# isarandi/metrabs

Measured on NVIDIA H100. Metric: crops/sec, higher is better.
Workload: dtype bf16

## Files before the change

### metrabs_b200/csrc/engine.cu

```cuda
#include "../../include/metrabs_b200.h"

#include <dlfcn.h>

#include <algorithm>
#include <cmath>
#include <cstdarg>
#include <cstdio>
#include <cstdlib>
#include <cstring>
#include <iterator>
#include <map>
#include <string>
#include <vector>

#include "common.cuh"
#include "conv_simt.cuh"
#include "decode.cuh"
#include "tc_gemm.cuh"
#include "tc_fmb.cuh"
#include "tc_tf32.cuh"
#include "dw_tma.cuh"
#include "multiperson.cuh"

using namespace mtb;
// ... 759 lines not shown
    if (pl.ok && pl.n_rb <= kPoolSlices) {
      op.dw_kernel = DW_TMA_DIL;
      op.dw_plan = pl;
      op.pool_slices = pl.n_rb;
    }
    return;
  }
  if (dw5x5_eligible(op)) {
    if (!is_tc16(h)) return;
    if (op.act != ACT_SILU) {
      op.dw_kernel = DW_5X5_16B;
      return;
    }
    op.dw_kernel = DW_5X5_POOL_16B;
    const int strips = op.Hout * ((op.Wout + kDw5OW - 1) / kDw5OW);
    const int groups = dw5_pool_shape(op.Cout).groups;
    op.pool_slices = std::min((strips + groups - 1) / groups, kPoolSlices);
    return;
  }
  if (!dw_strip_eligible(op)) return;
  if (is_tc16(h)) {
    if (op.stride == 1 && op.Hin == op.Hout && op.Win == op.Wout) {
      const DwTmaPlan pl = dw_tma_plan(op.Hout, op.Wout);
      if (pl.ok && pl.n_rb <= kPoolSlices) {
        op.dw_kernel = DW_TMA;
        op.dw_plan = pl;
        op.pool_slices = pl.n_rb;
        return;
      }
    }
    op.dw_kernel = DW_STRIP_16B;
  } else if (h->cfg.precision == MTB_PRECISION_TF32X3) {
    op.dw_kernel = DW_STRIP_F32;
  } else {
    return;
  }
  const int strips = op.Hout * ((op.Wout + kDwOW - 1) / kDwOW);
  op.pool_slices = std::min((strips + 7) / 8, kPoolSlices);
}

int op_class(const Op& op) {
  switch (op.type) {
    case OP_STEM: return KC_STEM;
    case OP_DW: return KC_DWCONV;
    case OP_POOL: return KC_POOL;
    case OP_MAXPOOL: return KC_OTHER;
    default: break;
  }
  if (op.small_io) return KC_SE_FC;
  if (op.fmb.ready) return KC_FMB;
  if (op.tc.ready) return KC_TC_GEMM;
  if (op.tc32.ready) return KC_TC32;
  return KC_IGEMM_SIMT;
}

double op_weight_bytes(const Op& op) {
  if (op.type == OP_POOL || op.type == OP_MAXPOOL) return 0.0;
  return (double)op.R * op.S * (op.depthwise ? 1 : op.Cin) * op.Cout * (op.tc.ready ? 2.0 : 4.0);
}

double op_bytes(const mtb_handle* h, const Op& op, int B) {
  const double es = op.small_io ? 4.0 : (double)elem_size(h);
  double in = (double)B * op.Hin * op.Win * op.Cin * (op.type == OP_STEM ? 4.0 : es);
  double out = (double)B * op.Hout * op.Wout * op.Cout * es;
  if (op.type == OP_POOL) out = (double)B * op.Cout * 4.0;
  double res = op.res_buf != BUF_NONE ? out : 0.0;
  return in + out + res + op_weight_bytes(op);
}

bool stem_fast_enabled() {
  static int v = -1;
  if (v < 0) {
    const char* e = getenv("MTB_STEM_FAST");
    v = (e && e[0] == '0') ? 0 : 1;
  }
  return v == 1;
}

template <typename T>
int run_op_t(mtb_handle* h, const Op& op, const float* crops, int B, const Workspace& ws, void* features,
             cudaStream_t st) {
  constexpr bool k16 = sizeof(T) == 2;
  if constexpr (k16) {
    if (op.type == OP_CONV && op.tc.ready && op.scale_buf != BUF_NONE) {
      void* x = buf_ptr(ws, op.in_buf, features);
      const double bytes = 2.0 * B * op.Hin * op.Win * op.Cin * elem_size(h);
      ProfScope ps(h, KC_SE_SCALE, 0.0, bytes, st, false);
      const char* e = tc_se_scale_launch<T>(x, (const float*)buf_ptr(ws, op.scale_buf, features), B, op.Hin * op.Win, op.Cin, st);
      if (e) return fail(h, MTB_ERR_CUDA, "se scale %s: %s", op.name.c_str(), e);
      h->launches++;
    }
  }
  ProfScope prof(h, op_class(op), op.flops * B, op_bytes(h, op, B), st);
  switch (op.type) {
    case OP_STEM: {
      StemParams p;
      p.in = crops;
      p.out = buf_ptr(ws, op.out_buf, features); p.w = op.d_w; p.bias = op.d_bias;
      for (int i = 0; i < 3; ++i) { p.pre_scale[i] = op.pre_scale[i]; p.pre_shift[i] = op.pre_shift[i]; }
      p.pre_scale[3] = 1.f; p.pre_shift[3] = 0.f;
      p.B = B; p.Hin = op.Hin; p.Win = op.Win; p.Cin = op.Cin; p.Hout = op.Hout; p.Wout = op.Wout; p.Cout = op.Cout;
      p.R = op.R; p.S = op.S; p.stride = op.stride; p.pad_t = op.pad_t; p.pad_l = op.pad_l; p.act = op.act;
      size_t smem = ((size_t)op.R * op.S * op.Cin + 1) * op.Cout * 4;
      const size_t pixels = (size_t)B * op.Hout * op.Wout;
      const bool effnet_stem = op.R == 3 && op.S == 3 && op.Cin == 3 && op.stride == 2 && stem_fast_enabled();
      if (effnet_stem && op.Cout == 32) launch_k(stem3x3s2_kernel<T, 32>, dim3(grid_for(pixels, 128)), dim3(128), (size_t)28 * 32 * 4, st, p);
      else if (effnet_stem && op.Cout == 24) launch_k(stem3x3s2_kernel<T, 24>, dim3(grid_for(pixels, 128)), dim3(128), (size_t)28 * 24 * 4, st, p);
      else if (op.Cout % 32 == 0) launch_k(stem_conv_wide_kernel<T, 32>, dim3(grid_for(pixels * (op.Cout / 32), 128)), dim3(128), smem, st, p);
      else if (op.Cout % 24 == 0) launch_k(stem_conv_wide_kernel<T, 24>, dim3(grid_for(pixels * (op.Cout / 24), 128)), dim3(128), smem, st, p);
      else if (op.Cout % 16 == 0) launch_k(stem_conv_wide_kernel<T, 16>, dim3(grid_for(pixels * (op.Cout / 16), 128)), dim3(128), smem, st, p);
      else launch_k(stem_conv_kernel<T>, dim3(grid_for(pixels * (op.Cout / 4), 256)), dim3(256), smem, st, p);
      h->launches++;
      break;
    }
    case OP_CONV:
    case OP_DW:
    case OP_MAXPOOL: {
      ConvParams p;
      p.in = buf_ptr(ws, op.in_buf, features);
      p.out = buf_ptr(ws, op.out_buf, features);
      p.res = buf_ptr(ws, op.res_buf, features);
      p.a_scale = (const float*)buf_ptr(ws, op.scale_buf, features);
      p.w = op.d_w; p.bias = op.d_bias;
      p.B = B; p.Hin = op.Hin; p.Win = op.Win; p.Cin = op.Cin; p.Hout = op.Hout; p.Wout = op.Wout; p.Cout = op.Cout;
      p.R = op.R; p.S = op.S; p.stride = op.stride; p.dil = op.dil; p.pad_t = op.pad_t; p.pad_l = op.pad_l; p.act = op.act;
      p.res_first = op.res_first ? 1 : 0;
      if (op.type == OP_DW) {
        float* pooled = op.fused_pool ? (float*)buf_ptr(ws, BUF_SMALL0, features) : nullptr;
        if (op.dw_kernel == DW_TMA || op.dw_kernel == DW_TMA_DIL || op.dw_kernel == DW_STRIP_16B) {
          if constexpr (!k16) {
            return fail(h, MTB_ERR_CUDA, "depthwise %s: 16-bit kernel chosen for fp32 storage", op.name.c_str());
          } else if (op.dw_kernel == DW_TMA || op.dw_kernel == DW_TMA_DIL) {
            const char* e = dw_tma_launch<T>(op.dw_maps, op.dw_plan, p.in, p.out, op.d_w, op.d_bias, pooled, B, op.Hout, op.Wout,
                                             op.Cout, op.pad_t, op.pad_l, op.act, op.dw_kernel == DW_TMA ? 1 : op.dil, st);
            if (e) return fail(h, MTB_ERR_CUDA, "depthwise (TMA) launch %s: %s", op.name.c_str(), e);
          } else {
            const dim3 grid((op.Cout / 8 + 31) / 32, op.pool_slices, B), block(32, 8);
            const cudaError_t e = dw_dispatch<ACT_SILU, ACT_RELU, ACT_HSWISH>(op, [&](auto s, auto a) {
              return launch_k(dwconv3x3_pool_16b_kernel<T, s, a, kDwOW>, grid, block, 0, st, p, pooled);
            });
            if (e != cudaSuccess) return fail(h, MTB_ERR_CUDA, "depthwise launch %s: %s", op.name.c_str(), cudaGetErrorString(e));
          }
        } else if (op.dw_kernel == DW_STRIP_F32) {
          const dim3 grid((op.Cout / 4 + 31) / 32, op.pool_slices, B), block(32, 8);
          const cudaError_t e = dw_dispatch<ACT_SILU, ACT_RELU, ACT_HSWISH>(op, [&](auto s, auto a) {
            return launch_k(dwconv3x3_pool_f32_kernel<s, a, kDwOW>, grid, block, 0, st, p, pooled);
          });
          if (e != cudaSuccess) return fail(h, MTB_ERR_CUDA, "depthwise launch %s: %s", op.name.c_str(), cudaGetErrorString(e));
        } else if (op.dw_kernel == DW_5X5_16B || op.dw_kernel == DW_5X5_POOL_16B) {
          if constexpr (!k16) {
            return fail(h, MTB_ERR_CUDA, "depthwise %s: 16-bit kernel chosen for fp32 storage", op.name.c_str());
          } else {
            cudaError_t e;
            if (op.dw_kernel == DW_5X5_16B) {
              const size_t items = (size_t)B * op.Hout * ((op.Wout + kDw5OW - 1) / kDw5OW) * (op.Cout / 8);
              const dim3 grid(grid_for(items, 256));
              e = dw_dispatch<ACT_RELU, ACT_HSWISH>(op, [&](auto s, auto a) {
                return launch_k(dwconv5x5_16b_kernel<T, s, a, kDw5OW>, grid, dim3(256), 0, st, p, nullptr);
              });
            } else {
              const Dw5PoolShape sh = dw5_pool_shape(op.Cout);
              const dim3 grid(sh.chunks, op.pool_slices, B), block(sh.cb * sh.groups);
              e = dw_dispatch<ACT_SILU>(op, [&](auto s, auto a) {
                return launch_k(dwconv5x5_16b_kernel<T, s, a, kDw5OW, true>, grid, block, 0, st, p, pooled);
              });
            }
            if (e != cudaSuccess) return fail(h, MTB_ERR_CUDA, "depthwise launch %s: %s", op.name.c_str(), cudaGetErrorString(e));
          }
        } else {
          size_t total = (size_t)B * op.Hout * op.Wout * (op.Cout / 4);
          launch_k(dwconv_kernel<T>, dim3(grid_for(total, 256)), dim3(256), 0, st, p);
        }
      } else if (op.type == OP_MAXPOOL) {
        size_t total = (size_t)B * op.Hout * op.Wout * (op.Cout / 4);
        launch_k(maxpool_kernel<T>, dim3(grid_for(total, 256)), dim3(256), 0, st, p);
      } else if (op.small_io) {
        if (op.pool_src > 0 && h->ops[op.pool_src].fused_pool) {
          p.a_splits = h->ops[op.pool_src - 1].pool_slices;
          p.a_split_stride = (size_t)B * op.Cin;
        }
        float* final_out = (float*)p.out;
        if (op.ksplit > 1) {
          p.ksplit = op.ksplit;
          p.out = buf_ptr(ws, BUF_SMALL0 + 2, features);
        }
        cudaError_t e = launch_conv_igemm<float, float>(p, st);
        if (e == cudaSuccess && op.ksplit > 1) {
          const int n = B * op.Cout;
          launch_k(se_reduce_kernel, dim3((n + 255) / 256), dim3(256), 0, st, (const float*)p.out, (const float*)op.d_bias, final_out, n,
                   op.Cout, op.ksplit, op.act);
          h->launches++;
          e = cudaGetLastError();
        }
        if (e != cudaSuccess) return fail(h, MTB_ERR_CUDA, "launch %s: %s", op.name.c_str(), cudaGetErrorString(e));
      } else if (op.tc.ready) {
        if constexpr (!k16) return fail(h, MTB_ERR_CUDA, "%s: tensor-core weights in an fp32 mode", op.name.c_str());
        else {
          const char* e = tc_conv_launch<T>(op.tc, p, op.res_first, st);
          if (e) return fail(h, MTB_ERR_CUDA, "tensor-core launch %s: %s", op.name.c_str(), e);
        }
      } else if (op.tc32.ready) {
        const char* e = tc32_conv_launch(op.tc32, p, op.res_first, st);
        if (e) return fail(h, MTB_ERR_CUDA, "3xTF32 launch %s: %s", op.name.c_str(), e);
      } else {
        cudaError_t e = launch_conv_igemm<T, T>(p, st);
        if (e != cudaSuccess) return fail(h, MTB_ERR_CUDA, "launch %s: %s", op.name.c_str(), cudaGetErrorString(e));
      }
      h->launches++;
      break;
    }
    case OP_POOL: {
      dim3 grid((op.Cin + 127) / 128, B), block(32, 8);
      launch_k(pool_mean_kernel<T>, dim3(grid), dim3(block), 0, st, (const T*)buf_ptr(ws, op.in_buf, features),
                                                   (float*)buf_ptr(ws, op.out_buf, features), op.Hin * op.Win, op.Cin);
      h->launches++;
      break;
    }
  }
  cudaError_t e = cudaGetLastError();
  if (e != cudaSuccess) return fail(h, MTB_ERR_CUDA, "launch %s: %s", op.name.c_str(), cudaGetErrorString(e));
  return MTB_OK;
}

int run_op(mtb_handle* h, const Op& op, const float* crops, int B, const Workspace& ws, void* features, cudaStream_t st) {
  if (op.type == OP_POOL && op.fused_pool) return MTB_OK;
  return with_storage(h, [&](auto* tag) { return run_op_t<std::remove_pointer_t<decltype(tag)>>(h, op, crops, B, ws, features, st); });
}

int run_fused_block(mtb_handle* h, const Op& a, const Op& b, int B, const Workspace& ws, void* features, cudaStream_t st) {
  const void* in = buf_ptr(ws, a.in_buf, features);
  void* out = buf_ptr(ws, b.out_buf, features);
  const double bytes = 2.0 * B * a.Hin * a.Win * (a.Cin + b.Cout) + 2.0 * (9.0 * a.Cin * a.Cout + (double)b.Cin * b.Cout);
  ProfScope prof(h, KC_FMB, (a.flops + b.flops) * B, bytes, st);
  const char* e = with_storage16(h, [&](auto* tag) {
    return fmb_launch<std::remove_pointer_t<decltype(tag)>>(a.fmb, in, out, B, a.Hin, a.Win, a.pad_t, a.pad_l, b.res_buf != BUF_NONE, st);
  });
  if (e) return fail(h, MTB_ERR_CUDA, "fused FusedMBConv launch %s: %s", a.name.c_str(), e);
  h->launches++;
  return MTB_OK;
}

int run_ops_range(mtb_handle* h, size_t first, size_t last, const float* crops, int B, const Workspace& ws, void* features,
                  cudaStream_t st) {
  for (size_t k = first; k < last; ++k) {
    h->prof_cur_op = (int)k;
    int rc;
    if (h->ops[k].fmb.ready && k + 1 < last) {
      rc = run_fused_block(h, h->ops[k], h->ops[k + 1], B, ws, features, st);
      ++k;
    } else {
      rc = run_op(h, h->ops[k], crops, B, ws, features, st);
    }
    if (rc) return rc;
  }
  h->prof_cur_op = -1;
  return MTB_OK;
}

int run_backbone(mtb_handle* h, const float* crops, int B, Workspace& ws, void* features, cudaStream_t st) {
  return run_ops_range(h, 0, h->ops.size(), crops, B, ws, features, st);
}

int check_common(mtb_handle* h, int B, size_t ws_bytes, const void* workspace) {
  if (!h) return fail(nullptr, MTB_ERR_INVALID_ARG, "null handle");
  if (!h->finalized) return fail(h, MTB_ERR_NOT_FINALIZED, "mtb_finalize_weights has not been called");
  if (B <= 0) return fail(h, MTB_ERR_INVALID_ARG, "batch must be positive (got %d)", B);
  if (!workspace || ws_bytes < layout(h, B, nullptr).total)
    return fail(h, MTB_ERR_WORKSPACE, "workspace too small: need %zu bytes for batch %d, got %zu",
                layout(h, B, nullptr).total, B, ws_bytes);
  return MTB_OK;
}

DecodeScale make_scale(const mtb_config& c) {
  DecodeScale s;
  int last = c.proc_side - 1;
  int last_rc = last - (last % c.stride_test);
  float add = 0.f;
  if (c.centered_stride) add += (float)(c.stride_test / 2);
  if (c.legacy_centered_stride_bug) add += (float)(c.stride_test / 2);
  s.img_mul = (float)last_rc;
// ... 1108 lines not shown
```

### metrabs_b200/csrc/tc_gemm.cuh

```cuda
#pragma once
#include <cuda.h>

#include <algorithm>
#include <cstdio>
#include <cstdlib>
#include <cstring>
#include <string>
#include <vector>

#include "common.cuh"
#include "conv_simt.cuh"
#include "decode.cuh"
#include "wgmma.cuh"

namespace mtb {

__device__ __forceinline__ uint32_t smem_u32(const void* p) { return (uint32_t)__cvta_generic_to_shared(p); }

__device__ __forceinline__ void mbar_init(uint64_t* bar, uint32_t count) {
  asm volatile("mbarrier.init.shared::cta.b64 [%0], %1;" ::"r"(smem_u32(bar)), "r"(count));
}
__device__ __forceinline__ void mbar_expect_tx(uint64_t* bar, uint32_t bytes) {
  asm volatile("mbarrier.arrive.expect_tx.shared::cta.b64 _, [%0], %1;" ::"r"(smem_u32(bar)), "r"(bytes) : "memory");
}
__device__ __forceinline__ void mbar_arrive(uint64_t* bar) {
  asm volatile("mbarrier.arrive.shared::cta.b64 _, [%0];" ::"r"(smem_u32(bar)) : "memory");
}
__device__ __forceinline__ bool mbar_try_wait(uint64_t* bar, uint32_t parity) {
  uint32_t ok;
  asm volatile(
      "{\n"
      ".reg .pred P1;\n"
      "mbarrier.try_wait.parity.shared::cta.b64 P1, [%1], %2;\n"
      "selp.u32 %0, 1, 0, P1;\n"
      "}\n"
      : "=r"(ok)
      : "r"(smem_u32(bar)), "r"(parity)
      : "memory");
  return ok != 0;
}
__device__ __forceinline__ void mbar_wait(uint64_t* bar, uint32_t parity) {
  if (mbar_try_wait(bar, parity)) return;
  const long long t0 = clock64();
  while (!mbar_try_wait(bar, parity))
    if (clock64() - t0 > 8000000000LL) __trap();
}
__device__ __forceinline__ void fence_barrier_init() { asm volatile("fence.mbarrier_init.release.cluster;" ::: "memory"); }
__device__ __forceinline__ void fence_proxy_async() { asm volatile("fence.proxy.async.shared::cta;" ::: "memory"); }
__device__ __forceinline__ void wg_sync(int wg) { asm volatile("bar.sync %0, 128;" ::"r"(1 + wg) : "memory"); }

__device__ __forceinline__ void tma_load_2d(void* dst, const CUtensorMap* map, uint64_t* bar, int c0, int c1) {
  asm volatile(
      "cp.async.bulk.tensor.2d.shared::cluster.global.tile.mbarrier::complete_tx::bytes [%0], [%1, {%3, %4}], [%2];" ::"r"(
          smem_u32(dst)),
      "l"(map), "r"(smem_u32(bar)), "r"(c0), "r"(c1)
      : "memory");
}
__device__ __forceinline__ void tma_load_4d(void* dst, const CUtensorMap* map, uint64_t* bar, int c0, int c1, int c2, int c3) {
  asm volatile(
      "cp.async.bulk.tensor.4d.shared::cluster.global.tile.mbarrier::complete_tx::bytes [%0], [%1, {%3, %4, %5, %6}], [%2];" ::"r"(
          smem_u32(dst)),
      "l"(map), "r"(smem_u32(bar)), "r"(c0), "r"(c1), "r"(c2), "r"(c3)
      : "memory");
}
__device__ __forceinline__ void tma_store_2d(const CUtensorMap* map, const void* src, int c0, int c1) {
  asm volatile("cp.async.bulk.tensor.2d.global.shared::cta.bulk_group [%0, {%2, %3}], [%1];" ::"l"(map), "r"(smem_u32(src)), "r"(c0),
               "r"(c1)
               : "memory");
}
__device__ __forceinline__ void tma_store_4d(const CUtensorMap* map, const void* src, int c0, int c1, int c2, int c3) {
  asm volatile("cp.async.bulk.tensor.4d.global.shared::cta.bulk_group [%0, {%2, %3, %4, %5}], [%1];" ::"l"(map), "r"(smem_u32(src)),
               "r"(c0), "r"(c1), "r"(c2), "r"(c3)
               : "memory");
}
__device__ __forceinline__ void bulk_commit() { asm volatile("cp.async.bulk.commit_group;" ::: "memory"); }
__device__ __forceinline__ void bulk_wait_read() { asm volatile("cp.async.bulk.wait_group.read 0;" ::: "memory"); }
__device__ __forceinline__ void bulk_wait() { asm volatile("cp.async.bulk.wait_group 0;" ::: "memory"); }
__device__ __forceinline__ void tma_prefetch_desc(const CUtensorMap* map) {
  asm volatile("prefetch.tensormap [%0];" ::"l"(map) : "memory");
}

template <int RB>
__device__ __forceinline__ uint64_t gmma_desc(uint32_t smem_addr) {
  uint64_t d = 0;
  d |= (uint64_t)((smem_addr & 0x3FFFF) >> 4);
  d |= (uint64_t)1 << 16;
  d |= (uint64_t)((8 * RB) >> 4) << 32;
  d |= (uint64_t)(RB == 128 ? 1 : 2) << 62;
  return d;
}

constexpr int TC_BM = 128, TC_BK = 64;
constexpr int TC_A_BYTES = TC_BM * TC_BK * 2;
constexpr int TC_THREADS = 288;
constexpr int TC_CONSUMER_WARPS = 8;
constexpr int TC_TILE_W = 16, TC_TILE_H = 8;
constexpr int TCP_THREADS = 384;

template <int BN>
struct TcRing {
  static constexpr int stages = BN >= 128 ? 5 : 8;
  static constexpr int stage_bytes = TC_A_BYTES + BN * TC_BK * 2;
  static constexpr int slab_cols = BN < 64 ? BN : 64;
  static constexpr int out_bytes = TC_BM * BN * 2;
  static constexpr int out_off = stages * stage_bytes;
  static constexpr int bar_off = out_off + 2 * out_bytes;
  static constexpr int smem_bytes = bar_off + 256  + 1024 ;
};

struct TcConvParams {
  const void* res;
  const float* bias;
  void* out;
  int mode;
  int Hin, Win;
  int M;
  int Cout, Cin;
  int kchunks, taps;
  int Hout, Wout, tiles_w, tiles_h, pad_t, pad_l, S, stride, dil;
  int m_tiles, n_tiles;
};

template <int R>
__device__ __forceinline__ void setmaxnreg_dec() { asm volatile("setmaxnreg.dec.sync.aligned.u32 %0;" ::"n"(R)); }
template <int R>
__device__ __forceinline__ void setmaxnreg_inc() { asm volatile("setmaxnreg.inc.sync.aligned.u32 %0;" ::"n"(R)); }
__device__ __forceinline__ void named_bar_sync(int id) { asm volatile("bar.sync %0, 256;" ::"r"(id) : "memory"); }
__device__ __forceinline__ void named_bar_arrive(int id) { asm volatile("bar.arrive %0, 256;" ::"r"(id) : "memory"); }

__device__ __forceinline__ float tanh_approx(float x) {
  float y;
  asm("tanh.approx.f32 %0, %1;" : "=f"(y) : "f"(x));
  return y;
}
template <int ACT, typename T = __nv_bfloat16>
__device__ __forceinline__ float tc_act(float x) {
  if constexpr (ACT == ACT_SILU && is_f16<T>) {
    return silu_f16out(x);
  } else if constexpr (ACT == ACT_SILU) {
    float h = 0.5f * x;
    return fmaf(h, tanh_approx(h), h);
  } else if constexpr (ACT == ACT_RELU) {
    return fmaxf(x, 0.0f);
  } else if constexpr (ACT == ACT_HSWISH) {
    return x * __saturatef(fmaf(x, 1.0f / 6.0f, 0.5f));
  } else {
    return x;
  }
}
__device__ __forceinline__ bool tile_row_offset(int mode, int m_blk, int r, int M, int Cout, int tiles_w, int tiles_h, int Hout, int Wout,
                                                size_t& off) {
  if (mode == 0) {
    const int m = m_blk * TC_BM + r;
    off = (size_t)m * Cout;
    return m < M;
  }
  const int tw = m_blk % tiles_w, th = (m_blk / tiles_w) % tiles_h, b = m_blk / (tiles_w * tiles_h);
  const int oh = th * TC_TILE_H + (r >> 4), ow = tw * TC_TILE_W + (r & 15);
  off = ((size_t)(b * Hout + oh) * Wout + ow) * Cout;
  return oh < Hout && ow < Wout;
// ... 14 lines not shown
template <typename P>
__device__ __forceinline__ void tma_load_tap_boxes(uint8_t* dst, int box_bytes, const CUtensorMap* map, uint64_t* bar, const P& p, int m_blk,
                                                   int kc) {
  const int tw = m_blk % p.tiles_w, th = (m_blk / p.tiles_w) % p.tiles_h, b = m_blk / (p.tiles_w * p.tiles_h);
  for (int s = 0; s < p.S; ++s)
    tma_load_4d(dst + s * box_bytes, map, bar, kc * TC_BK, tw * TC_TILE_W - p.pad_l + s, th * TC_TILE_H - p.pad_t, b);
}

template <typename T, int ACT, int RES, int BN>
__device__ __forceinline__ void tc_tile_epilogue(const float* acc, uint8_t* stg, const CUtensorMap* tmO, const TcConvParams& p, int m_blk,
                                                 int n_blk, int c) {
  constexpr int SW = BN < 64 ? BN : 64, RB = SW * 2;
  typedef typename Pair16<T>::type T2;
  const T* __restrict__ res = (const T*)p.res;
  const int warp = (threadIdx.x >> 5) & 3, lane = threadIdx.x & 31;
  const bool leader = (threadIdx.x & 127) == 0;
  if (leader) bulk_wait_read();
  wg_sync(2 + c);
  const int c0 = n_blk * BN + 2 * (lane & 3);
#pragma unroll
  for (int mh = 0; mh < 2; ++mh) {
    const float* accm = acc + mh * (BN / 2);
#pragma unroll
    for (int h = 0; h < 2; ++h) {
      const int r = mh * 64 + warp * 16 + (lane >> 2) + 8 * h;
      size_t off = 0;
      if constexpr (RES != 0) {
        if (!tile_row_offset(p.mode, m_blk, r, p.M, p.Cout, p.tiles_w, p.tiles_h, p.Hout, p.Wout, off)) continue;
      }
      const uint32_t swz = RB == 128 ? (uint32_t)(r & 7) : (uint32_t)((r >> 1) & 3);
      constexpr int JB = BN / 8 < 8 ? BN / 8 : 8;
#pragma unroll
      for (int j0 = 0; j0 < BN / 8; j0 += JB) {
        T2 rv2[RES != 0 ? JB : 1];
        if constexpr (RES != 0) {
#pragma unroll
          for (int jj = 0; jj < JB; ++jj)
            if (c0 + 8 * (j0 + jj) < p.Cout) rv2[jj] = *reinterpret_cast<const T2*>(res + off + c0 + 8 * (j0 + jj));
        }
#pragma unroll
        for (int j = j0; j < j0 + JB; ++j) {
          const int cc = c0 + 8 * j;
          if (cc >= p.Cout) break;
          const float2 bv = __ldg(reinterpret_cast<const float2*>(p.bias + cc));
          float o0 = accm[4 * j + 2 * h] + bv.x, o1 = accm[4 * j + 2 * h + 1] + bv.y;
          if constexpr (RES != 0) {
            const float2 rv = Pair16<T>::unpack(rv2[j - j0]);
            if constexpr (RES == 2) {
              o0 = tc_act<ACT, T>(o0 + rv.x);
              o1 = tc_act<ACT, T>(o1 + rv.y);
            } else {
              o0 = tc_act<ACT, T>(o0) + rv.x;
              o1 = tc_act<ACT, T>(o1) + rv.y;
            }
          } else {
            o0 = tc_act<ACT, T>(o0);
            o1 = tc_act<ACT, T>(o1);
          }
          const int col = 8 * j + 2 * (lane & 3), cs = col % SW;
          const uint32_t o = (uint32_t)(col / SW) * (TC_BM * RB) + (uint32_t)r * RB + ((((uint32_t)cs >> 3) ^ swz) << 4) + (cs & 7) * 2;
          *reinterpret_cast<T2*>(stg + o) = Pair16<T>::pack(o0, o1);
        }
      }
    }
  }
  fence_proxy_async();
  wg_sync(2 + c);
  if (leader) {
#pragma unroll
    for (int sl = 0; sl < BN / SW; ++sl) {
      const int col0 = n_blk * BN + sl * SW;
      if (col0 >= p.Cout) break;
      if (p.mode == 0) {
        tma_store_2d(tmO, stg + sl * TC_BM * RB, col0, m_blk * TC_BM);
      } else {
        const int tw = m_blk % p.tiles_w, th = (m_blk / p.tiles_w) % p.tiles_h, b = m_blk / (p.tiles_w * p.tiles_h);
        tma_store_4d(tmO, stg + sl * TC_BM * RB, col0, tw * TC_TILE_W, th * TC_TILE_H, b);
      }
    }
    bulk_commit();
  }
}

template <typename T, int ACT, int RES, int BN>
__global__ void __launch_bounds__(TCP_THREADS, 1)
tc_conv_kernel(const __grid_constant__ CUtensorMap tmA, const __grid_constant__ CUtensorMap tmB, const __grid_constant__ CUtensorMap tmO,
               const TcConvParams p) {
  using Ring = TcRing<BN>;
  constexpr int STAGES = Ring::stages;
  extern __shared__ uint8_t tc_smem_raw[];
  uint8_t* smem = (uint8_t*)(((uintptr_t)tc_smem_raw + 1023) & ~(uintptr_t)1023);
  uint64_t* full = (uint64_t*)(smem + Ring::bar_off);
  uint64_t* empty = full + STAGES;

  const int wg = threadIdx.x >> 7, lane = threadIdx.x & 31;
  if (threadIdx.x == 0) {
    tma_prefetch_desc(&tmA);
    tma_prefetch_desc(&tmB);
    tma_prefetch_desc(&tmO);
    for (int i = 0; i < STAGES; ++i) {
      mbar_init(&full[i], 1);
      mbar_init(&empty[i], 4);
    }
    fence_barrier_init();
  }
  __syncthreads();

  const int tiles = p.m_tiles * p.n_tiles;
  const int num_kb = p.taps * p.kchunks;
  if (wg == 0) {
    setmaxnreg_dec<40>();
    if (threadIdx.x == 0) {
      int it = 0;
      for (int t = blockIdx.x; t < tiles; t += gridDim.x) {
        const int m_blk = t / p.n_tiles, n_blk = t - m_blk * p.n_tiles;
        for (int kb = 0; kb < num_kb; ++kb, ++it) {
          const int s = it % STAGES;
          mbar_wait(&empty[s], ((it / STAGES) & 1) ^ 1);
          uint8_t* sa = smem + s * Ring::stage_bytes;
          const int tap = kb / p.kchunks, kc = kb - tap * p.kchunks;
          mbar_expect_tx(&full[s], Ring::stage_bytes);
          tma_load_a_tile<TC_BK>(sa, &tmA, &full[s], p, m_blk, kb);
          tma_load_2d(sa + TC_A_BYTES, &tmB, &full[s], tap * p.Cin + kc * TC_BK, n_blk * BN);
        }
      }
    }
    return;
  }
  setmaxnreg_inc<232>();
  const int c = wg - 1;
  for (int i = c, t = blockIdx.x + c * gridDim.x; t < tiles; i += 2, t += 2 * gridDim.x) {
    const int m_blk = t / p.n_tiles, n_blk = t - m_blk * p.n_tiles;
    float acc[BN];
#pragma unroll
    for (int q = 0; q < BN; ++q) acc[q] = 0.f;
    if (t != (int)blockIdx.x) named_bar_sync(1 + c);
    int it = i * num_kb, prev = -1;
    for (int kb = 0; kb < num_kb; ++kb, ++it) {
      const int s = it % STAGES;
      mbar_wait(&full[s], (it / STAGES) & 1);
      const uint32_t a = smem_u32(smem + s * Ring::stage_bytes);
      const uint32_t b = smem_u32(smem + s * Ring::stage_bytes + TC_A_BYTES);
      wgmma_fence();
#pragma unroll
      for (int k = 0; k < TC_BK / 16; ++k) {
        const uint64_t db = gmma_desc<128>(b + 32 * k);
        wgmma_16b<T, BN>(acc, gmma_desc<128>(a + 32 * k), db, (uint32_t)(kb | k));
        wgmma_16b<T, BN>(acc + BN / 2, gmma_desc<128>(a + 64 * 128 + 32 * k), db, (uint32_t)(kb | k));
      }
      wgmma_commit();
      wgmma_wait<1>();
      if (prev >= 0) {
        __syncwarp();
        if (lane == 0) mbar_arrive(&empty[prev]);
      }
      prev = s;
    }
    wgmma_wait<0>();
    wgmma_fence_regs<BN>(acc);
    __syncwarp();
    if (lane == 0) mbar_arrive(&empty[prev]);
    if (t + (int)gridDim.x < tiles) named_bar_arrive(2 - c);
    tc_tile_epilogue<T, ACT, RES, BN>(acc, smem + Ring::out_off + c * Ring::out_bytes, &tmO, p, m_blk, n_blk, c);
  }
  if ((threadIdx.x & 127) == 0) bulk_wait();
}

template <int CK>
struct Tc3x3Smem {
  static constexpr int RB = CK * 2;
  static constexpr int w_tap_bytes = CK * RB;
  static constexpr int box_bytes = TC_TILE_W * (TC_TILE_H + 2) * RB;
  static constexpr int sets = CK == 32 ? 2 : 1;
  static constexpr int box_off = 9 * w_tap_bytes;
  static constexpr int out_bytes = TC_BM * CK * 2;
  static constexpr int out_off = box_off + 2 * sets * 3 * box_bytes;
  static constexpr int bar_off = out_off + 2 * out_bytes;
  static constexpr int smem_bytes = bar_off + 256  + 1024 ;
};

inline bool tc3x3s1_eligible(int R, int S, int stride, int dil, int cin, int cout, int act) {
  return R == 3 && S == 3 && stride == 1 && dil == 1 && cin <= 64 && cout <= 64 && cin % 8 == 0 && cout % 8 == 0 &&
         (act == ACT_SILU || act == ACT_RELU);
}
inline int tc3x3s1_width(int cin, int cout) { return std::max(cin, cout) <= 32 ? 32 : 64; }

template <typename T, int ACT, int RES, int CK>
__global__ void __launch_bounds__(TCP_THREADS, 1)
tc_conv3x3s1_kernel(const __grid_constant__ CUtensorMap tmA, const __grid_constant__ CUtensorMap tmB,
                    const __grid_constant__ CUtensorMap tmO, const TcConvParams p) {
  using L = Tc3x3Smem<CK>;
  constexpr int BN = CK, SETS = L::sets, RB = L::RB;
  extern __shared__ uint8_t tc_smem_raw[];
  uint8_t* smem = (uint8_t*)(((uintptr_t)tc_smem_raw + 1023) & ~(uintptr_t)1023);
  uint64_t* w_full = (uint64_t*)(smem + L::bar_off);
  uint64_t* box_full = w_full + 1;
  uint64_t* box_empty = box_full + 2 * SETS;

  const int wg = threadIdx.x >> 7, lane = threadIdx.x & 31;
  if (threadIdx.x == 0) {
    tma_prefetch_desc(&tmA);
    tma_prefetch_desc(&tmB);
    tma_prefetch_desc(&tmO);
    mbar_init(w_full, 1);
    for (int i = 0; i < 2 * SETS; ++i) {
      mbar_init(&box_full[i], 1);
      mbar_init(&box_empty[i], 4);
    }
    fence_barrier_init();
  }
  __syncthreads();

  const int tiles = p.m_tiles;
  if (wg == 0) {
    setmaxnreg_dec<40>();
    if (threadIdx.x == 0) {
      mbar_expect_tx(w_full, 9 * L::w_tap_bytes);
      for (int tap = 0; tap < 9; ++tap) tma_load_2d(smem + tap * L::w_tap_bytes, &tmB, w_full, tap * p.Cin, 0);
      int n = 0;
      for (int t = blockIdx.x; t < tiles; t += gridDim.x, ++n) {
        const int j = n >> 1, b = (n & 1) * SETS + j % SETS;
        mbar_wait(&box_empty[b], ((j / SETS) & 1) ^ 1);
        mbar_expect_tx(&box_full[b], 3 * L::box_bytes);
// ... 114 lines not shown
  std::vector<Entry> entries;
  size_t replaced = 0;

  template <typename Encode, typename... K>
  const char* get(const CUtensorMap** maps, Encode&& encode, K... key) {
    static_assert(sizeof...(K) <= kKeyWords, "TmapCache key too long");
    Entry n = {};
    int i = 0;
    ((n.key[i++] = key_word(key)), ...);
    for (const Entry& e : entries)
      if (std::equal(e.key, e.key + kKeyWords, n.key)) {
        *maps = e.map;
        return nullptr;
      }
    if (const char* err = encode(n.map)) return err;
    Entry& slot = entries.size() < kEntries ? entries.emplace_back(n) : (entries[replaced++ % kEntries] = n);
    *maps = slot.map;
    return nullptr;
  }
  template <typename X>
  static uint64_t key_word(X x) {
    if constexpr (std::is_pointer<X>::value) return (uint64_t)(uintptr_t)x;
    else return (uint64_t)x;
  }
};

inline const char* upload_dev(std::vector<void*>& allocs, void** dev, const void* host, size_t bytes) {
  cudaError_t e = cudaMalloc(dev, bytes);
  if (e == cudaSuccess) {
    allocs.push_back(*dev);
    e = cudaMemcpy(*dev, host, bytes, cudaMemcpyHostToDevice);
  }
  return e == cudaSuccess ? nullptr : cudaGetErrorString(e);
}

struct TcWeights {
  bool ready = false;
  void* d_w = nullptr;
  float* d_bias = nullptr;
  int Cout = 0, Cin = 0, taps = 1, S = 1;
  int n_real = 0;
  mutable TmapCache maps;
};

inline bool tc_eligible(bool is_conv, bool depthwise, bool small_io, int k, int stride, int cin, int cout) {
  if (!is_conv || depthwise || small_io) return false;
  if (cin % 8 != 0 || cout % 8 != 0) return false;
  return (stride == 1 || stride == 2) && (k == 1 || k == 3);
}

inline __nv_bfloat16 host_bf16(float f) {
  uint32_t u;
  memcpy(&u, &f, 4);
  uint32_t lsb = (u >> 16) & 1u;
  u += 0x7FFFu + lsb;
  uint16_t h = (uint16_t)(u >> 16);
  __nv_bfloat16 out;
  memcpy(&out, &h, 2);
  return out;
}

inline __half host_f16(float f) { return __float2half_rn(f); }
template <typename T>
inline T host_16b(float f) {
  if constexpr (std::is_same<T, __half>::value) return host_f16(f);
  else return host_bf16(f);
}

template <typename T>
inline const char* tc_prepare_weights(TcWeights& w, const float* wk, const float* bias, int K, int cout, int R, int S, int cin,
                                      std::vector<void*>& allocs) {
  std::vector<T> t((size_t)K * cout);
  for (int k = 0; k < K; ++k)
    for (int n = 0; n < cout; ++n) t[(size_t)n * K + k] = host_16b<T>(wk[(size_t)k * cout + n]);
  const char* e = upload_dev(allocs, &w.d_w, t.data(), t.size() * sizeof(T));
  if (!e) e = upload_dev(allocs, (void**)&w.d_bias, bias, (size_t)cout * 4);
  if (e) return e;
  w.Cout = cout; w.Cin = cin; w.taps = R * S; w.S = S;
  w.ready = true;
  return nullptr;
}

inline int tc_pick_bn(int cout) { return cout <= 32 ? 32 : cout <= 64 ? 64 : 128; }

template <typename T>
inline const char* tc_conv_launch(const TcWeights& w, const ConvParams& p, bool res_first, cudaStream_t st) {
  TcConvParams q;
  q.res = p.res; q.bias = w.d_bias; q.out = p.out;
  q.mode = (p.R == 1 && p.stride == 1) ? 0 : 1;
  q.Hin = p.Hin; q.Win = p.Win;
  q.Cout = p.Cout; q.Cin = p.Cin;
  q.taps = w.taps; q.S = w.S; q.stride = p.stride; q.dil = p.dil;
  q.kchunks = (p.Cin + TC_BK - 1) / TC_BK;
  q.Hout = p.Hout; q.Wout = p.Wout; q.pad_t = p.pad_t; q.pad_l = p.pad_l;
  q.tiles_w = (p.Wout + TC_TILE_W - 1) / TC_TILE_W;
  q.tiles_h = (p.Hout + TC_TILE_H - 1) / TC_TILE_H;
  q.M = p.B * p.Hout * p.Wout;
  const bool s1 = tc3x3s1_eligible(p.R, p.S, p.stride, p.dil, p.Cin, p.Cout, p.act);
  const int bn = s1 ? tc3x3s1_width(p.Cin, p.Cout) : tc_pick_bn(p.Cout);
  q.m_tiles = q.mode == 0 ? (q.M + TC_BM - 1) / TC_BM : p.B * q.tiles_w * q.tiles_h;
  q.n_tiles = (p.Cout + bn - 1) / bn;
  const CUtensorMap* m = nullptr;
  const char* e = w.maps.get(&m, [&](CUtensorMap* c) {
    const CUtensorMapSwizzle sw = CU_TENSOR_MAP_SWIZZLE_128B;
    const uint32_t slab = (uint32_t)std::min(bn, 64);
    const CUtensorMapSwizzle out_sw = slab == 64 ? sw : CU_TENSOR_MAP_SWIZZLE_64B;
    const char* r;
    if (s1) {
      r = make_tmap_nhwc<T>(&c[0], p.in, p.B, p.Hin, p.Win, p.Cin, bn, TC_TILE_W, TC_TILE_H + 2, 1, 1, out_sw);
      if (!r) r = make_tmap_2d<T>(&c[1], w.d_w, p.Cout, (uint64_t)w.taps * p.Cin, bn, bn, out_sw);
    } else {
      r = q.mode == 0 ? make_tmap_2d<T>(&c[0], p.in, q.M, p.Cin, TC_BM, TC_BK, sw)
                      : make_tmap_nhwc<T>(&c[0], p.in, p.B, p.Hin, p.Win, p.Cin, TC_BK, TC_TILE_W, TC_TILE_H, 1, p.stride, sw);
      if (!r) r = make_tmap_2d<T>(&c[1], w.d_w, p.Cout, (uint64_t)w.taps * p.Cin, bn, TC_BK, sw);
    }
    if (!r)
      r = q.mode == 0 ? make_tmap_2d<T>(&c[2], p.out, q.M, p.Cout, TC_BM, slab, out_sw)
                      : make_tmap_nhwc<T>(&c[2], p.out, p.B, p.Hout, p.Wout, p.Cout, slab, TC_TILE_W, TC_TILE_H, 1, 1, out_sw);
    return r;
  }, p.in, p.out, w.d_w, p.B, p.Hin, p.Win, p.Cin, p.Hout, p.Wout, p.Cout, w.taps, p.stride, bn, s1);
  if (e) return e;
  const dim3 grid(std::min(q.m_tiles * q.n_tiles, num_sms()));
  const int res_mode = p.res ? (res_first ? 2 : 1) : 0;
  if (s1)
    return with_const<ACT_SILU, ACT_RELU>(p.act, "unsupported activation in tc_conv3x3s1_kernel", [&](auto act) {
      return with_const<0, 1, 2>(res_mode, "unsupported residual mode", [&](auto res) {
        return with_const<32, 64>(bn, "unsupported width of tc_conv3x3s1_kernel", [&](auto ck) {
          return launch_smem(tc_conv3x3s1_kernel<T, act, res, ck>, grid, dim3(TCP_THREADS), Tc3x3Smem<ck>::smem_bytes, st, m[0], m[1], m[2],
                             q);
        });
      });
    });
  return with_const<ACT_NONE, ACT_SILU, ACT_RELU, ACT_HSWISH>(p.act, "unsupported activation in the tensor-core epilogue", [&](auto act) {
    return with_const<0, 1, 2>(res_mode, "unsupported residual mode", [&](auto res) {
      return with_const<32, 64, 128>(bn, "unsupported N tile", [&](auto bn_) {
        return launch_smem(tc_conv_kernel<T, act, res, bn_>, grid, dim3(TCP_THREADS), TcRing<bn_>::smem_bytes, st, m[0], m[1], m[2], q);
      });
    });
  });
}

template <typename T>
inline const char* tc_se_scale_launch(void* x, const float* s, int B, int P, int C, cudaStream_t st) {
  size_t total8 = (size_t)B * P * C / 8;
  launch_k(se_scale_kernel<T>, dim3(grid_for(total8, 256)), dim3(256), 0, st, (T*)x, s, P, C, total8);
  cudaError_t e = cudaGetLastError();
  return e == cudaSuccess ? nullptr : cudaGetErrorString(e);
}

struct TcHeadParams {
  float4* states;
  const float* bias;
  int B, P, W, n_out, C;
  int bnp;
  int cpt;
  int npt;
  int m_tiles;
  int kblocks;
};
constexpr int TCH_STAGES = 2;
constexpr int TCH_STAGE_BYTES = TC_A_BYTES + 256 * TC_BK * 2;
constexpr int TCH_STG_OFF = TCH_STAGES * TCH_STAGE_BYTES;
constexpr int TCH_BAR_OFF = TCH_STG_OFF + 128 * 256 * 4;
constexpr int TCH_SMEM_BYTES = TCH_BAR_OFF + 64 + 1024 ;

__device__ __forceinline__ uint32_t tch_stg(int row, int col) {
  return (uint32_t)(row * 256 + ((((col >> 2) ^ (row & 7))) << 2) + (col & 3)) * 4u;
}

template <typename T>
__global__ void __launch_bounds__(TC_THREADS, 1)
tc_head_kernel(const __grid_constant__ CUtensorMap tmW, const __grid_constant__ CUtensorMap tmF, const TcHeadParams p) {
  extern __shared__ uint8_t tc_smem_raw[];
  uint8_t* smem = (uint8_t*)(((uintptr_t)tc_smem_raw + 1023) & ~(uintptr_t)1023);
  uint64_t* full = (uint64_t*)(smem + TCH_BAR_OFF);
  uint64_t* empty = full + TCH_STAGES;
  float* stg = (float*)(smem + TCH_STG_OFF);

  const int warp = threadIdx.x >> 5, lane = threadIdx.x & 31;
  if (threadIdx.x == TC_CONSUMER_WARPS * 32) {
    tma_prefetch_desc(&tmW);
    tma_prefetch_desc(&tmF);
    for (int i = 0; i < TCH_STAGES; ++i) {
      mbar_init(&full[i], 1);
      mbar_init(&empty[i], TC_CONSUMER_WARPS);
    }
    fence_barrier_init();
  }
  __syncthreads();

  const int g = blockIdx.x / p.m_tiles, m_blk = blockIdx.x - g * p.m_tiles;
  const int n_kb = p.npt * p.kblocks;
  if (warp == TC_CONSUMER_WARPS) {
    if (lane == 0) {
      const uint32_t stage_tx = TC_A_BYTES + (uint32_t)p.bnp * TC_BK * 2;
      for (int i = 0; i < n_kb; ++i) {
        const int s = i % TCH_STAGES, pt = i / p.kblocks, kb = i - pt * p.kblocks;
        mbar_wait(&empty[s], ((i / TCH_STAGES) & 1) ^ 1);
        uint8_t* sa = smem + s * TCH_STAGE_BYTES;
        const int row0 = p.cpt > 0 ? g * p.bnp : g * p.P + pt * p.bnp;
        mbar_expect_tx(&full[s], stage_tx);
        tma_load_2d(sa, &tmW, &full[s], kb * TC_BK, m_blk * TC_BM);
        tma_load_2d(sa + TC_A_BYTES, &tmF, &full[s], kb * TC_BK, row0);
      }
    }
    return;
  }
  const int wg = warp >> 2, tid = threadIdx.x & 127;
  const int row = wg * 64 + tid;
  const int n = m_blk * TC_BM + row;
  const bool owner = tid < 64;
  const bool nvalid = owner && n < p.n_out;
  const float bias_n = nvalid ? p.bias[n] : 0.f;
  constexpr float L2E = 1.4426950408889634f;
  int crop = p.cpt > 0 ? g * p.cpt : g;
  int pix = 0, x = 0, y = 0;
  float m = -INFINITY, mL = -INFINITY, s_ = 0.f, sx = 0.f, sy = 0.f;
  int i = 0;
  for (int pt = 0; pt < p.npt; ++pt) {
// ... 186 lines not shown
```

Before: 6676.

## Fuse squeeze-excitation channel scaling into the tensor-core 1x1 projection GEMM

```diff
diff --git a/metrabs_b200/csrc/engine.cu b/metrabs_b200/csrc/engine.cu
--- a/metrabs_b200/csrc/engine.cu
+++ b/metrabs_b200/csrc/engine.cu
@@ -865,7 +865,7 @@
              cudaStream_t st) {
   constexpr bool k16 = sizeof(T) == 2;
   if constexpr (k16) {
-    if (op.type == OP_CONV && op.tc.ready && op.scale_buf != BUF_NONE) {
+    if (op.type == OP_CONV && op.tc.ready && op.scale_buf != BUF_NONE && !tc_se_in_gemm(op.Cout)) {
       void* x = buf_ptr(ws, op.in_buf, features);
       const double bytes = 2.0 * B * op.Hin * op.Win * op.Cin * elem_size(h);
       ProfScope ps(h, KC_SE_SCALE, 0.0, bytes, st, false);
@@ -979,6 +979,7 @@
       } else if (op.tc.ready) {
         if constexpr (!k16) return fail(h, MTB_ERR_CUDA, "%s: tensor-core weights in an fp32 mode", op.name.c_str());
         else {
+          if (!tc_se_in_gemm(op.Cout)) p.a_scale = nullptr;
           const char* e = tc_conv_launch<T>(op.tc, p, op.res_first, st);
           if (e) return fail(h, MTB_ERR_CUDA, "tensor-core launch %s: %s", op.name.c_str(), e);
         }
diff --git a/metrabs_b200/csrc/tc_gemm.cuh b/metrabs_b200/csrc/tc_gemm.cuh
--- a/metrabs_b200/csrc/tc_gemm.cuh
+++ b/metrabs_b200/csrc/tc_gemm.cuh
@@ -46,6 +46,14 @@
     if (clock64() - t0 > 8000000000LL) __trap();
 }
 __device__ __forceinline__ void fence_barrier_init() { asm volatile("fence.mbarrier_init.release.cluster;" ::: "memory"); }
+__device__ __forceinline__ uint4 ld_shared_u4(uint32_t addr) {
+  uint4 v;
+  asm volatile("ld.shared.v4.u32 {%0, %1, %2, %3}, [%4];" : "=r"(v.x), "=r"(v.y), "=r"(v.z), "=r"(v.w) : "r"(addr) : "memory");
+  return v;
+}
+__device__ __forceinline__ void st_shared_u4(uint32_t addr, const uint4& v) {
+  asm volatile("st.shared.v4.u32 [%0], {%1, %2, %3, %4};" ::"r"(addr), "r"(v.x), "r"(v.y), "r"(v.z), "r"(v.w) : "memory");
+}
 __device__ __forceinline__ void fence_proxy_async() { asm volatile("fence.proxy.async.shared::cta;" ::: "memory"); }
 __device__ __forceinline__ void wg_sync(int wg) { asm volatile("bar.sync %0, 128;" ::"r"(1 + wg) : "memory"); }
 
@@ -76,6 +84,7 @@
 __device__ __forceinline__ void bulk_commit() { asm volatile("cp.async.bulk.commit_group;" ::: "memory"); }
 __device__ __forceinline__ void bulk_wait_read() { asm volatile("cp.async.bulk.wait_group.read 0;" ::: "memory"); }
 __device__ __forceinline__ void bulk_wait() { asm volatile("cp.async.bulk.wait_group 0;" ::: "memory"); }
+__device__ __forceinline__ void prefetch_l1(const void* p) { asm volatile("prefetch.global.L1 [%0];" ::"l"(p)); }
 __device__ __forceinline__ void tma_prefetch_desc(const CUtensorMap* map) {
   asm volatile("prefetch.tensormap [%0];" ::"l"(map) : "memory");
 }
@@ -256,16 +265,96 @@
   }
 }
 
-template <typename T, int ACT, int RES, int BN>
+struct SeRows {
+  int r0, r1;
+  int ca, cb;
+};
+__device__ __forceinline__ SeRows se_rows(int u, int m0, int M, int P) {
+  const int g = u >> 3;
+  SeRows w;
+  w.r0 = 10 * g + min(g, 8);
+  w.r1 = min(w.r0 + (g < 8 ? 11 : 10), M - m0);
+  w.ca = (m0 + w.r0) / P;
+  w.cb = (m0 + max(w.r1, w.r0 + 1) - 1) / P;
+  return w;
+}
+template <typename T>
+__device__ __forceinline__ void se_scale_chunk(uint32_t addr, const float4& s0, const float4& s1) {
+  typedef typename Pair16<T>::type T2;
+  uint4 v = ld_shared_u4(addr);
+  T2* v2 = reinterpret_cast<T2*>(&v);
+  float2 f = Pair16<T>::unpack(v2[0]);
+  v2[0] = Pair16<T>::pack(f.x * s0.x, f.y * s0.y);
+  f = Pair16<T>::unpack(v2[1]);
+  v2[1] = Pair16<T>::pack(f.x * s0.z, f.y * s0.w);
+  f = Pair16<T>::unpack(v2[2]);
+  v2[2] = Pair16<T>::pack(f.x * s1.x, f.y * s1.y);
+  f = Pair16<T>::unpack(v2[3]);
+  v2[3] = Pair16<T>::pack(f.x * s1.z, f.y * s1.w);
+  st_shared_u4(addr, v);
+}
+template <typename T>
+__device__ __forceinline__ void se_scale_rows(uint32_t a, int L, int rb, int re, const float4& s0, const float4& s1) {
+  typedef typename Pair16<T>::type T2;
+  int r = rb;
+#pragma unroll 1
+  for (; r + 1 < re; r += 2) {
+    const uint32_t p0 = a + r * 128 + ((L ^ (r & 7)) << 4), p1 = a + (r + 1) * 128 + ((L ^ ((r + 1) & 7)) << 4);
+    uint4 v = ld_shared_u4(p0), w = ld_shared_u4(p1);
+    T2* v2 = reinterpret_cast<T2*>(&v);
+    T2* w2 = reinterpret_cast<T2*>(&w);
+#pragma unroll
+    for (int j = 0; j < 4; ++j) {
+      const float sx = j < 2 ? (j == 0 ? s0.x : s0.z) : (j == 2 ? s1.x : s1.z);
+      const float sy = j < 2 ? (j == 0 ? s0.y : s0.w) : (j == 2 ? s1.y : s1.w);
+      const float2 f = Pair16<T>::unpack(v2[j]), g = Pair16<T>::unpack(w2[j]);
+      v2[j] = Pair16<T>::pack(f.x * sx, f.y * sy);
+      w2[j] = Pair16<T>::pack(g.x * sx, g.y * sy);
+    }
+    st_shared_u4(p0, v);
+    st_shared_u4(p1, w);
+  }
+  if (r < re) se_scale_chunk<T>(a + r * 128 + ((L ^ (r & 7)) << 4), s0, s1);
+}
+template <typename T>
+__device__ __forceinline__ void se_scale_a_tile(uint32_t a, uint64_t* full, uint32_t ph, const SeRows& w, const float* __restrict__ s, int m0,
+                                                int P, int Cin, int kb, int u) {
+  const int L = u & 7, k = kb * TC_BK + 8 * L;
+  if (k >= Cin || w.r1 <= w.r0) {
+    mbar_wait(full, ph);
+    return;
+  }
+  const float4* sa = reinterpret_cast<const float4*>(s + (size_t)w.ca * Cin + k);
+  const float4* sb = reinterpret_cast<const float4*>(s + (size_t)w.cb * Cin + k);
+  const float4 a0 = __ldg(sa), a1 = __ldg(sa + 1), b0 = __ldg(sb), b1 = __ldg(sb + 1);
+  if (k + TC_BK < Cin) {
+    prefetch_l1(sa + TC_BK / 4);
+    prefetch_l1(sb + TC_BK / 4);
+  }
+  mbar_wait(full, ph);
+  const int ra = min((w.ca + 1) * P - m0, w.r1);
+  const int rb = max(min(w.cb * P - m0, w.r1), ra);
+  se_scale_rows<T>(a, L, w.r0, ra, a0, a1);
+#pragma unroll 1
+  for (int r = ra; r < rb; ++r) {
+    const float4* sr = reinterpret_cast<const float4*>(s + (size_t)((m0 + r) / P) * Cin + k);
+    se_scale_chunk<T>(a + r * 128 + ((L ^ (r & 7)) << 4), __ldg(sr), __ldg(sr + 1));
+  }
+  se_scale_rows<T>(a, L, rb, w.r1, b0, b1);
+}
+
+template <typename T, int ACT, int RES, int BN, bool SE = false>
 __global__ void __launch_bounds__(TCP_THREADS, 1)
 tc_conv_kernel(const __grid_constant__ CUtensorMap tmA, const __grid_constant__ CUtensorMap tmB, const __grid_constant__ CUtensorMap tmO,
-               const TcConvParams p) {
+               const TcConvParams p, const float* __restrict__ a_scale) {
   using Ring = TcRing<BN>;
   constexpr int STAGES = Ring::stages;
   extern __shared__ uint8_t tc_smem_raw[];
   uint8_t* smem = (uint8_t*)(((uintptr_t)tc_smem_raw + 1023) & ~(uintptr_t)1023);
   uint64_t* full = (uint64_t*)(smem + Ring::bar_off);
   uint64_t* empty = full + STAGES;
+  uint64_t* ready = empty + STAGES;
+  uint64_t* landed = SE ? ready : full;
 
   const int wg = threadIdx.x >> 7, lane = threadIdx.x & 31;
   if (threadIdx.x == 0) {
@@ -275,15 +364,16 @@
     for (int i = 0; i < STAGES; ++i) {
       mbar_init(&full[i], 1);
       mbar_init(&empty[i], 4);
+      if constexpr (SE) mbar_init(&ready[i], 3);
     }
     fence_barrier_init();
   }
   __syncthreads();
 
   const int tiles = p.m_tiles * p.n_tiles;
-  const int num_kb = p.taps * p.kchunks;
+  const int num_kb = SE ? p.kchunks : p.taps * p.kchunks;
   if (wg == 0) {
-    setmaxnreg_dec<40>();
+    setmaxnreg_dec<SE ? 56 : 40>();
     if (threadIdx.x == 0) {
       int it = 0;
       for (int t = blockIdx.x; t < tiles; t += gridDim.x) {
@@ -298,10 +388,26 @@
           tma_load_2d(sa + TC_A_BYTES, &tmB, &full[s], tap * p.Cin + kc * TC_BK, n_blk * BN);
         }
       }
+    } else if constexpr (SE) {
+      if (threadIdx.x >= 32) {
+        const int u = threadIdx.x - 32, P = p.Hin * p.Win;
+        int it = 0;
+        for (int t = blockIdx.x; t < tiles; t += gridDim.x) {
+          const int m0 = (t / p.n_tiles) * TC_BM;
+          const SeRows w = se_rows(u, m0, p.M, P);
+          for (int kb = 0; kb < num_kb; ++kb, ++it) {
+            const int s = it % STAGES;
+            se_scale_a_tile<T>(smem_u32(smem + s * Ring::stage_bytes), &full[s], (it / STAGES) & 1, w, a_scale, m0, P, p.Cin, kb, u);
+            fence_proxy_async();
+            __syncwarp();
+            if (lane == 0) mbar_arrive(&ready[s]);
+          }
+        }
+      }
     }
     return;
   }
-  setmaxnreg_inc<232>();
+  setmaxnreg_inc<SE ? 224 : 232>();
   const int c = wg - 1;
   for (int i = c, t = blockIdx.x + c * gridDim.x; t < tiles; i += 2, t += 2 * gridDim.x) {
     const int m_blk = t / p.n_tiles, n_blk = t - m_blk * p.n_tiles;
@@ -312,7 +418,7 @@
     int it = i * num_kb, prev = -1;
     for (int kb = 0; kb < num_kb; ++kb, ++it) {
       const int s = it % STAGES;
-      mbar_wait(&full[s], (it / STAGES) & 1);
+      mbar_wait(&landed[s], (it / STAGES) & 1);
       const uint32_t a = smem_u32(smem + s * Ring::stage_bytes);
       const uint32_t b = smem_u32(smem + s * Ring::stage_bytes + TC_A_BYTES);
       wgmma_fence();
@@ -593,6 +699,7 @@
 }
 
 inline int tc_pick_bn(int cout) { return cout <= 32 ? 32 : cout <= 64 ? 64 : 128; }
+inline bool tc_se_in_gemm(int cout) { return cout <= 256; }
 
 template <typename T>
 inline const char* tc_conv_launch(const TcWeights& w, const ConvParams& p, bool res_first, cudaStream_t st) {
@@ -607,6 +714,8 @@
   q.tiles_w = (p.Wout + TC_TILE_W - 1) / TC_TILE_W;
   q.tiles_h = (p.Hout + TC_TILE_H - 1) / TC_TILE_H;
   q.M = p.B * p.Hout * p.Wout;
+  if (p.a_scale && (q.mode != 0 || !tc_se_in_gemm(p.Cout)))
+    return "squeeze-excitation scale outside the 1x1 projections tc_conv_kernel scales (tc_se_in_gemm)";
   const bool s1 = tc3x3s1_eligible(p.R, p.S, p.stride, p.dil, p.Cin, p.Cout, p.act);
   const int bn = s1 ? tc3x3s1_width(p.Cin, p.Cout) : tc_pick_bn(p.Cout);
   q.m_tiles = q.mode == 0 ? (q.M + TC_BM - 1) / TC_BM : p.B * q.tiles_w * q.tiles_h;
@@ -642,10 +751,20 @@
         });
       });
     });
+  if (p.a_scale)
+    return with_const<ACT_NONE>(p.act, "unsupported activation with a squeeze-excitation scale", [&](auto act) {
+      return with_const<0, 1>(res_mode, "unsupported residual mode with a squeeze-excitation scale", [&](auto res) {
+        return with_const<32, 64, 128>(bn, "unsupported N tile", [&](auto bn_) {
+          return launch_smem(tc_conv_kernel<T, act, res, bn_, true>, grid, dim3(TCP_THREADS), TcRing<bn_>::smem_bytes, st, m[0], m[1], m[2],
+                             q, p.a_scale);
+        });
+      });
+    });
   return with_const<ACT_NONE, ACT_SILU, ACT_RELU, ACT_HSWISH>(p.act, "unsupported activation in the tensor-core epilogue", [&](auto act) {
     return with_const<0, 1, 2>(res_mode, "unsupported residual mode", [&](auto res) {
       return with_const<32, 64, 128>(bn, "unsupported N tile", [&](auto bn_) {
-        return launch_smem(tc_conv_kernel<T, act, res, bn_>, grid, dim3(TCP_THREADS), TcRing<bn_>::smem_bytes, st, m[0], m[1], m[2], q);
+        return launch_smem(tc_conv_kernel<T, act, res, bn_>, grid, dim3(TCP_THREADS), TcRing<bn_>::smem_bytes, st, m[0], m[1], m[2], q,
+                           (const float*)nullptr);
       });
     });
   });
```

New measurement: 6899 (median of 6 runs). 3.3% higher.
